# Janmajayamall/tfhe-research

Measured on AMD Instinct MI355X. Metric: programmable_bootstraps_per_sec, higher is better.
Workload: dtype f64

## Files before the change

tfhe-research_amd/csrc/pbs_wave.h:

```cpp
#pragma once
#include "wave_ntt.h"

namespace tfhe {

template <int V>
struct IntC {
  static constexpr int value = V;
};

template <int I, int END, class F>
TFHE_HD void static_for(F&& f) {
  if constexpr (I < END) {
    f(IntC<I>{});
    static_for<I + 1, END>(f);
  }
}

template <class F, int LOGN, int K>
constexpr int key_layout_e() {
  return (F::kLogShrink == 1 && LOGN == 9 && K == 1) ? 8 : 0;
}

struct PbsParams {
  u32 n;
  u32 k;
  u32 log_n;
  u32 tv_shift;
  u32 log_base;
  u32 levels;
  u32 ignored_bits;
  u32 first_shift;
  u32 acc_glwe = 0;
  u32 acc_offset = 0;
};

struct KsParams {
  u32 log_base;
  u32 levels;
  u32 ignored_bits;
  u32 first_shift;
};

TFHE_HD u32 round_value(u32 v, u32 ignored_bits) {
  if (ignored_bits == 0) return v;
  return ((v >> ignored_bits) + ((v >> (ignored_bits - 1)) & 1u)) << ignored_bits;
}

struct RoundConsts {
  u32 half, keep;
};
TFHE_HD RoundConsts round_consts(u32 ignored_bits) {
  return ignored_bits == 0 ? RoundConsts{0u, ~0u} : RoundConsts{1u << (ignored_bits - 1), ~((1u << ignored_bits) - 1u)};
}
TFHE_HD u32 round_value_fast(u32 v, RoundConsts rc) { return (v + rc.half) & rc.keep; }

TFHE_HD u32 decompose_limb(u32 v, u32 shift, u32 log_base, u32& carry) {
  const u32 res = ((v >> shift) & ((1u << log_base) - 1u)) + carry;
  const u32 carry_mask = res & (1u << (log_base - 1));
  carry = carry_mask >> (log_base - 1);
  return res - (carry_mask << 1);
}

template <bool SMALL_BASE>
TFHE_HD u32 decompose_limb_fast(u32& v, u32 shift, u32 log_base, u32 carry_width) {
  const u32 half = 1u << (log_base - 1);
#if defined(__HIP_DEVICE_COMPILE__)
  const u32 res = __builtin_amdgcn_ubfe(v, shift, log_base) + __builtin_amdgcn_ubfe(v, log_base - 1, carry_width);
  const u32 hb = res & half;
  u32 digit;
  if (SMALL_BASE) {
    asm("v_mad_i32_i24 %0, %1, -2, %2" : "=v"(digit) : "v"(hb), "v"(res));
  } else {
    digit = res - (hb << 1);
  }
  asm("v_bfi_b32 %0, %1, %2, %3" : "=v"(v) : "s"(half), "v"(res), "v"(v));
  return digit;
#else
  const u32 cin = carry_width ? ((v >> (log_base - 1)) & 1u) : 0u;
  const u32 res = ((v >> shift) & ((1u << log_base) - 1u)) + cin;
  const u32 hb = res & half;
  v = hb | (v & ~half);
  return res - (hb << 1);
#endif
}

TFHE_HD u32 switch_modulus_2n(u32 v, u32 log_n) {
  const u32 sh = 32u - (log_n + 1u);
  return ((v >> sh) + ((v >> (sh - 1u)) & 1u)) & ((2u << log_n) - 1u);
}

template <int LOGN>
TFHE_HD u32 monomial_coeff(const u32* poly, int j, u32 m) {
  constexpr int N = 1 << LOGN;
  const int deg = (int)(m & (N - 1));
  const u32 flip = (m >> LOGN) & 1u;
  const u32 v = poly[(j - deg) & (N - 1)];
  const u32 negate = flip ^ (u32)(j < deg);
  return negate ? (0u - v) : v;
}

template <class F, int LOGN, int K, int G, int KEYS, int NS, class Ctx, class Src, class Out, class EndKey>
TFHE_HD void external_product_team_multi(const Ctx& c, const PbsParams& P, const typename F::elem* ggsw,
                                         size_t ggsw_words, Src src, Out out, EndKey end_of_key) {
  typedef typename F::elem elem;
  static_assert(KEYS == 1 || NS == 1, "several keys or several samples, not both");
  constexpr int LT = LOGN - F::kLogShrink;
  constexpr int E = NttShape<LT, G>::kE;
  constexpr int EC = NttShape<LOGN, G>::kE;
  constexpr int CO = F::kCoeffs;
  static_assert(EC == E * CO, "coefficients per lane");
  constexpr int T = NttShape<LOGN, G>::kThreads;
  constexpr int N = 1 << LT;
  constexpr int PARTS = F::kParts;
  const int lane = c.tid();
  const int me = c.group();
  constexpr bool SPLIT = F::template split_accum<E>() && KEYS == 1 && NS == 1;
  constexpr int ACCS = KEYS * PARTS;

  elem accum[NS][ACCS][E];
  elem accum_lo[SPLIT ? ACCS : 1][SPLIT ? E : 1];
#pragma unroll
  for (int s = 0; s < NS; ++s)
#pragma unroll
    for (int q = 0; q < ACCS; ++q)
#pragma unroll
      for (int r = 0; r < E; ++r) {
        accum[s][q][r] = SPLIT ? F::accum_init() : F::zero();
        if (SPLIT) accum_lo[SPLIT ? q : 0][SPLIT ? r : 0] = F::zero();
      }

  TopConsts<F, LT, G, true> ftop;
  ftop.issue(c.twiddles_uniform());
  u32 v[NS][EC];
  const RoundConsts rc = round_consts(P.ignored_bits);
#pragma unroll
  for (int s = 0; s < NS; ++s)
#pragma unroll
    for (int r = 0; r < EC; ++r) v[s][r] = round_value_fast(src(s, r * T + lane), rc);
  ftop.ready();

  constexpr int kChunkRegisters = 8;
  constexpr int TILES = (K + 1) * ACCS;
  constexpr int CH_MAX = kChunkRegisters * 8 / (int)sizeof(elem) / (NS > 1 ? 2 : 1);
  constexpr int CH = E < CH_MAX ? E : CH_MAX;
  constexpr int CHUNKS = TILES * (E / CH);
  auto tile_ptr = [&](u32 level, int sp, int a) -> const elem* {
    const int m = a / PARTS, q = a % PARTS;
    if (TFHE_PROBE_HOT_KEY) return ggsw;
    return ggsw + (size_t)m * ggsw_words + (((size_t)(sp * P.levels + level) * (K + 1) + me) * PARTS + q) * N;
  };
  const bool two = NS == 1 && c.exchange_buffers() == 2;
  elem kbuf[2][CH];
  constexpr bool OWN = F::kLogShrink == 1 && NS == 1 && G == 1 && !SPLIT;
  constexpr bool OWN_REGS = OWN;
  constexpr bool LATE = OWN;
  auto source_of = [&](int sp) -> int {
    if (!OWN) return sp;
    const int at = me + sp;
    return at > K ? at - (K + 1) : at;
  };
  auto load_chunk = [&](u32 level, auto ci_c, int buf) {
    constexpr int ci = decltype(ci_c)::value;
    constexpr int PIECES = E / CH;
    constexpr int q = ci % ACCS, r0 = ((ci / ACCS) % PIECES) * CH, src_poly = ci / (ACCS * PIECES);
    const elem* tile = tile_ptr(level, source_of(src_poly), q);
#pragma unroll
    for (int r = 0; r < CH; ++r)
      kbuf[buf][r] = tile[TFHE_PROBE_HOT_KEY ? (lane & 63) + r : spectrum_slot<LT, G, (int)sizeof(elem), key_layout_e<F, LOGN, K>()>(lane, r0 + r)];
  };
  auto buffers_of_level = [&](u32 t, Ctx (&cl)[NS]) {
#pragma unroll
    for (int s = 0; s < NS; ++s) cl[s] = c.with_exchange_buffer(NS > 1 ? s : (two ? (int)(t & 1u) : 0));
  };
#pragma unroll 1
  for (u32 t = 0; t < P.levels; ++t) {
    const u32 level = P.levels - 1 - t;
    const u32 shift = P.first_shift + P.log_base * t;
    Ctx cl[NS];
    buffers_of_level(t, cl);
    static_for<0, 1>([&](auto pre_c) { load_chunk(level, pre_c, decltype(pre_c)::value); });
    c.compiler_fence();
    constexpr int FS = 1;
    const u32 carry_width = (t == 0) ? 0u : 1u;
    elem own[OWN_REGS ? NS : 1][OWN_REGS ? E : 1];
#pragma unroll
    for (int s0 = 0; s0 < NS; s0 += FS) {
      elem work[FS][E];
      if (F::kMaxLogBase <= 23 || P.log_base <= 23) {
#pragma unroll
        for (int s = 0; s < FS; ++s)
#pragma unroll
          for (int r = 0; r < E; ++r) {
            u32 dg[CO];
#pragma unroll
            for (int q = 0; q < CO; ++q) dg[q] = decompose_limb_fast<true>(v[s0 + s][r + q * E], shift, P.log_base, carry_width);
            work[s][r] = F::from_digits(dg);
          }
      } else {
#pragma unroll
        for (int s = 0; s < FS; ++s)
#pragma unroll
          for (int r = 0; r < E; ++r) {
            u32 dg[CO];
#pragma unroll
            for (int q = 0; q < CO; ++q) dg[q] = decompose_limb_fast<false>(v[s0 + s][r + q * E], shift, P.log_base, carry_width);
            work[s][r] = F::from_digits(dg);
          }
      }
      Ctx cf[FS];
#pragma unroll
      for (int s = 0; s < FS; ++s) cf[s] = cl[s0 + s];
      if constexpr (LATE) {
        ntt_forward_multi<F, LT, G, true, true>(cf, work, ftop, [&]() { if (t > 0 && !two && s0 == 0) c.team_sync(); });
      } else {
        ntt_forward_multi<F, LT, G, true, true>(cf, work, ftop);
      }
#pragma unroll
      for (int s = 0; s < FS; ++s) {
        if (F::kReduceSpectrum) {
#pragma unroll
          for (int r = 0; r < E; ++r) work[s][r] = F::reduce(work[s][r]);
        }
        elem* mine = cf[s].scratch();
#pragma unroll
        for (int r = 0; r < E; ++r) mine[exchange_slot<LT, G>(lane, r)] = work[s][r];
        if constexpr (OWN_REGS) {
#pragma unroll
          for (int r = 0; r < E; ++r) own[s0 + s][r] = work[s][r];
        }
      }
    }
    if constexpr (!OWN) c.team_sync();
    elem d[NS][CH];
    constexpr bool MAC_LOW = mac_lowers_priority<elem, E>() && KEYS == 1;
    if constexpr (MAC_LOW) wave_priority<0>();
    static_for<0, CHUNKS>([&](auto ci_c) {
      constexpr int ci = decltype(ci_c)::value;
      constexpr int PIECES = E / CH;
      constexpr int q = ci % ACCS, r0 = ((ci / ACCS) % PIECES) * CH, sp = ci / (ACCS * PIECES);
      constexpr int cur = ci % 2;
      if constexpr (OWN && ci == ACCS * PIECES) c.team_sync();
      if constexpr (ci + 1 < CHUNKS) load_chunk(level, IntC<ci + 1>{}, (ci + 1) % 2);
      if constexpr (OWN_REGS && sp == 0) {
        if constexpr (q == 0) {
#pragma unroll
          for (int s = 0; s < NS; ++s)
#pragma unroll
            for (int r = 0; r < CH; ++r) d[s][r] = own[s][r0 + r];
        }
      } else if constexpr (q == 0 && !(TFHE_PROBE_NO_EXCHANGE_READS)) {
#pragma unroll
        for (int s = 0; s < NS; ++s) {
          const elem* spec = cl[s].scratch_of(source_of(sp));
#pragma unroll
          for (int r = 0; r < CH; ++r) d[s][r] = spec[exchange_slot<LT, G>(lane, r0 + r)];
        }
      } else if constexpr (q == 0 && ci == 0) {
#pragma unroll
        for (int s = 0; s < NS; ++s)
#pragma unroll
          for (int r = 0; r < CH; ++r) d[s][r] = kbuf[0][r];
      }
      c.compiler_fence();
#pragma unroll
      for (int s = 0; s < NS; ++s)
#pragma unroll
        for (int r = 0; r < CH; ++r) {
          if (SPLIT)
            F::mac(d[s][r], kbuf[cur][r], accum[s][q][r0 + r], accum_lo[SPLIT ? q : 0][SPLIT ? r0 + r : 0]);
          else
            accum[s][q][r0 + r] = F::mul_add(d[s][r], kbuf[cur][r], accum[s][q][r0 + r]);
        }
    });
    if constexpr (MAC_LOW) wave_priority<2>();
    if (!two && !LATE) c.team_sync();
  }

  Ctx ci[NS];
  buffers_of_level(P.levels, ci);
  TopConsts<F, LT, G, false> itop;
  itop.issue(c.twiddles_uniform());
  constexpr bool PAIR = NS == 1 && PARTS == 2 && G == 1 && !SPLIT && NttShape<LT, G>::kPasses == 3 && F::kLogShrink == 1 && E == 8;
  static_for<0, KEYS>([&](auto key_c) {
    constexpr int m = decltype(key_c)::value;
    if constexpr (PAIR) {
#pragma unroll
      for (int r = 0; r < E; ++r) {
        accum[0][m * PARTS][r] = F::before_inverse(accum[0][m * PARTS][r]);
        accum[0][m * PARTS + 1][r] = F::before_inverse(accum[0][m * PARTS + 1][r]);
      }
      if constexpr (m == 0) itop.ready();
      if constexpr (LATE && m == 0)
        ntt_inverse_pair<F, LT, G>(ci[0], accum[0][m * PARTS], accum[0][m * PARTS + 1], itop, [&]() { if (!two) c.team_sync(); });
      else
        ntt_inverse_pair<F, LT, G>(ci[0], accum[0][m * PARTS], accum[0][m * PARTS + 1], itop);
    }
    static_for<0, PAIR ? 0 : PARTS>([&](auto part_c) {
      constexpr int q = m * PARTS + decltype(part_c)::value;
      elem x[NS][E];
#pragma unroll
      for (int s = 0; s < NS; ++s)
#pragma unroll
        for (int r = 0; r < E; ++r)
          x[s][r] = SPLIT ? F::mac_finish(accum[s][q][r], accum_lo[SPLIT ? q : 0][SPLIT ? r : 0])
                          : F::before_inverse(accum[s][q][r]);
      if constexpr (LATE) {
        if constexpr (q == 0) {
          itop.ready();
          ntt_inverse_multi<F, LT, G>(ci, x, itop, [&]() { if (!two) c.team_sync(); });
        } else {
          ntt_inverse_multi<F, LT, G>(ci, x, itop);
        }
      } else {
        if constexpr (q == 0) itop.ready();
        ntt_inverse_multi<F, LT, G>(ci, x, itop);
      }
#pragma unroll
      for (int s = 0; s < NS; ++s)
#pragma unroll
        for (int r = 0; r < E; ++r) accum[s][q][r] = x[s][r];
    });
#pragma unroll
    for (int s = 0; s < NS; ++s)
#pragma unroll
      for (int r = 0; r < E; ++r) {
        elem parts[PARTS];
#pragma unroll
        for (int q = 0; q < PARTS; ++q) parts[q] = accum[s][m * PARTS + q][r];
        u32 vals[CO];
        F::finish(parts, vals);
#pragma unroll
        for (int q = 0; q < CO; ++q) out(m, s, (r + q * E) * T + lane, vals[q]);
      }
    end_of_key(m);
  });
  if (two) c.team_sync();
}

template <class F, int LOGN, int K, int G, int KEYS, class Ctx, class Src, class Out, class EndKey>
TFHE_HD void external_product_team_keys(const Ctx& c, const PbsParams& P, const typename F::elem* ggsw,
                                        size_t ggsw_words, Src src, Out out, EndKey end_of_key) {
  external_product_team_multi<F, LOGN, K, G, KEYS, 1>(
      c, P, ggsw, ggsw_words, [&](int, int j) -> u32 { return src(j); },
      [&](int m, int, int j, u32 value) { out(m, j, value); }, end_of_key);
}

template <class F, int LOGN, int K, int G, class Ctx, class Src, class Out>
TFHE_HD void external_product_team(const Ctx& c, const PbsParams& P, const typename F::elem* ggsw,
                                   Src src, Out out) {
  external_product_team_keys<F, LOGN, K, G, 1>(
      c, P, ggsw, 0, src, [&](int, int j, u32 value) { out(j, value); }, [](int) {});
}

template <class F, int LOGN, int K, int G, class Ctx>
TFHE_HD void pack_lwe_team(const Ctx& c, const PbsParams& P, const u32* masks_t, u32 d, const u32* body,
                           const typename F::elem* key , u32 slice_begin, u32 slice_end) {
  constexpr int E = NttShape<LOGN, G>::kE;
  constexpr int T = NttShape<LOGN, G>::kThreads;
  constexpr int N = 1 << LOGN;
  const int lane = c.tid();
  const int me = c.group();
  u32* acc = c.acc();
#pragma unroll
  for (int r = 0; r < E; ++r) acc[r * T + lane] = (me == K && body != nullptr) ? body[r * T + lane] : 0u;
  const size_t slice_words = (size_t)(K + 1) * P.levels * (K + 1) * F::kParts * (N >> F::kLogShrink);
#pragma unroll 1
  for (u32 s = slice_begin; s < slice_end; ++s) {
    const u32 i = c.uniform(s * (u32)(K + 1) + (u32)me);
    const bool live = i < d;
    const u32* column = masks_t + (size_t)(live ? i : 0u) * N;
    auto src = [&](int j) -> u32 { return live ? column[j] : 0u; };
    auto out = [&](int j, u32 value) { c.lds_add(acc + j, 0u - value); };
    external_product_team<F, LOGN, K, G>(c, P, key + (size_t)s * slice_words, src, out);
    if (G > 1 && c.exchange_buffers() != 2) c.poly_sync();
  }
}

struct RotateInit {
  int deg;
  u32 flip;
};
template <int LOGN>
TFHE_HD RotateInit rotate_init(const PbsParams& P, u32 body) {
  constexpr u32 N = 1u << LOGN;
  const u32 b_tilde = switch_modulus_2n(body, LOGN);
  const u32 m = (2u * N - b_tilde + 2u * N - P.acc_offset) & (2u * N - 1u);
  return RotateInit{(int)(m & (N - 1)), (m >> LOGN) & 1u};
}
template <int LOGN>
TFHE_HD u32 rotate_init_word(const RotateInit& ri, const u32* poly, int j, u32 shift) {
  constexpr int N = 1 << LOGN;
  const u32 t = poly[(j - ri.deg) & (N - 1)] << shift;
  return (ri.flip ^ (u32)(j < ri.deg)) ? (0u - t) : t;
}
template <int LOGN, int K, int COUNT, class Index>
TFHE_HD void rotate_init_fill(const PbsParams& P, const RotateInit& ri, const u32* tv, int me, u32* acc, Index index) {
  constexpr int N = 1 << LOGN;
  if (P.acc_glwe) {
    const u32* mine = tv + (size_t)me * N;
#pragma unroll
    for (int r = 0; r < COUNT; ++r) acc[index(r)] = rotate_init_word<LOGN>(ri, mine, index(r), 0u);
  } else {
#pragma unroll
    for (int r = 0; r < COUNT; ++r) acc[index(r)] = me == K ? rotate_init_word<LOGN>(ri, tv, index(r), P.tv_shift) : 0u;
  }
}

template <class F, int LOGN, int K, int G, int NS, class Ctx>
TFHE_HD void blind_rotate_team_multi(const Ctx& c, const PbsParams& P, const u32* const* lwe ,
                                     const u32* const* tv ,
                                     const typename F::elem* bsk , u32 i_begin, u32 i_end,
                                     const u32* const* resume ) {
  constexpr int E = NttShape<LOGN, G>::kE;
  constexpr int T = NttShape<LOGN, G>::kThreads;
  constexpr int N = 1 << LOGN;
  const int lane = c.tid();
  const int me = c.group();

  if (i_begin > 0) {
#pragma unroll
    for (int s = 0; s < NS; ++s) {
      u32* acc = c.acc(s);
      const u32* from = resume[s] + (size_t)me * N;
#pragma unroll
      for (int r = 0; r < E; ++r) acc[r * T + lane] = from[r * T + lane];
    }
  } else {
#pragma unroll
  for (int s = 0; s < NS; ++s) {
    u32* acc = c.acc(s);
    const RotateInit ri = rotate_init<LOGN>(P, lwe[s][P.n]);
    rotate_init_fill<LOGN, K, E>(P, ri, tv[s], me, acc, [&](int r) { return r * T + lane; });
  }
  }
  c.poly_sync();

  const size_t ggsw_words = (size_t)(K + 1) * P.levels * (K + 1) * F::kParts * (N >> F::kLogShrink);
#pragma unroll 1
  for (u32 i = i_begin; i < i_end; ++i) {
    u32 a_tilde[NS];
#pragma unroll
    for (int s = 0; s < NS; ++s) a_tilde[s] = c.uniform(switch_modulus_2n(lwe[s][i], LOGN));
    auto src = [&](int s, int j) -> u32 {
      const u32* acc = c.acc(s);
      return monomial_coeff<LOGN>(acc, j, a_tilde[s]) - acc[j];
    };
    auto out = [&](int, int s, int j, u32 value) { c.lds_add(c.acc(s) + j, value); };
    external_product_team_multi<F, LOGN, K, G, 1, NS>(c, P, bsk + (size_t)i * ggsw_words, 0, src, out, [](int) {});
    if (NS > 1 || c.exchange_buffers() != 2) c.poly_sync();
  }
}

template <class F, int LOGN, int K, int G, int NS, class Ctx>
TFHE_HD void blind_rotate_team_multi(const Ctx& c, const PbsParams& P, const u32* const* lwe, const u32* const* tv,
                                     const typename F::elem* bsk) {
  blind_rotate_team_multi<F, LOGN, K, G, NS>(c, P, lwe, tv, bsk, 0u, P.n, nullptr);
}

template <class F, int LOGN, int K, int G, class Ctx>
TFHE_HD void blind_rotate_team(const Ctx& c, const PbsParams& P, const u32* lwe ,
                               const u32* tv ,
                               const typename F::elem* bsk ) {
  const u32* const lwes[1] = {lwe};
  const u32* const tvs[1] = {tv};
  blind_rotate_team_multi<F, LOGN, K, G, 1>(c, P, lwes, tvs, bsk);
}

template <class F, int LOGN, int K, int LEVELS, int RING>
struct WideKeyRing {
  static constexpr int E = NttShape<LOGN - 1, 1>::kE;
  static constexpr int R = (K + 1) * LEVELS;
  static constexpr int kRing = RING;
  static_assert(LEVELS > 0 && RING > 0 && R % RING == 0, "the ring holds a divisor of the product's rows");
  typename F::elem slot[RING][E];
  template <int M>
  TFHE_HD void load(const typename F::elem* ggsw, int me, int q, int lane) {
    constexpr int level = M / (K + 1), sp = M % (K + 1);
    const typename F::elem* tile = ggsw + ((((size_t)sp * LEVELS + level) * (K + 1) + me) * 2 + q) * ((size_t)1 << (LOGN - 1));
#pragma unroll
    for (int r = 0; r < E; ++r)
      slot[M % RING][r] = tile[spectrum_slot<LOGN - 1, 1, (int)sizeof(typename F::elem), key_layout_e<F, LOGN, K>()>(lane, r)];
  }
  TFHE_HD void prime(const typename F::elem* ggsw, int me, int q, int lane) {
    static_for<0, RING>([&](auto m_c) { load<decltype(m_c)::value>(ggsw, me, q, lane); });
  }
};
struct NoKeyRing {
  static constexpr int kRing = 1;
};
constexpr int largest_divisor_upto(int n, int cap) {
  int best = 1;
  for (int d = 1; d <= n && d <= cap; ++d)
    if (n % d == 0) best = d;
  return best;
}
template <int LOGN, int K, int LEVELS>
constexpr int wide_ring_rows() {
  constexpr int E = NttShape<LOGN - 1, 1>::kE;
  return LEVELS == 0 ? 0 : largest_divisor_upto((K + 1) * LEVELS, (K == 1 ? 224 : 112) / (4 * E));
}


template <class F, int LOGN, int K, int LEVELS = 0, class Ring = NoKeyRing, class Ctx, class Src, class Out>
TFHE_HD void external_product_team_wide(const Ctx& c, const PbsParams& P, const typename F::elem* ggsw,
                                        const typename F::elem* ggsw_next, Ring& ring, Src src, Out out) {
  typedef typename F::elem elem;
  static_assert(F::kParts == 2 && F::kLogShrink == 1 && F::kCoeffs == 2, "the complex transform: two key parts, two coefficients per element");
  constexpr int LT = LOGN - 1;
  constexpr int E = NttShape<LT, 1>::kE;
  constexpr int EC = 2 * E;
  constexpr int T = 64;
  constexpr int N = 1 << LT;
  constexpr bool RINGED = LEVELS > 0;
  const int lane = c.tid();
  const int me = c.group();
  const int q = c.half();
  const u32 levels = RINGED ? (u32)LEVELS : P.levels;
  const u32 split = (levels + 1u) / 2u;
  const u32 t_begin = q == 0 ? 0u : split, t_end = q == 0 ? split : levels;

  TopConsts<F, LT, 1, true> ftop;
  ftop.issue(c.twiddles_uniform());
  u32 v[EC];
  const RoundConsts rc = round_consts(P.ignored_bits);
#pragma unroll
  for (int r = 0; r < EC; ++r) v[r] = round_value_fast(src(r * T + lane), rc);
  ftop.ready();

  constexpr int CH0 = E < 4 ? E : 4;
  constexpr int CH = (((K + 1) * (E / CH0)) % 2 == 0) ? CH0 : CH0 / 2;
  constexpr int PIECES = E / CH;
  constexpr int CHK = (K + 1) * PIECES;
  elem kbuf[RINGED ? 1 : 2][RINGED ? 1 : CH];
  auto load_chunk = [&](u32 level, auto ci_c, int buf) {
    constexpr int ci = decltype(ci_c)::value;
    constexpr int sp = ci / PIECES, r0 = (ci % PIECES) * CH;
    const elem* tile = ggsw + ((((size_t)sp * levels + level) * (K + 1) + me) * 2 + q) * N;
#pragma unroll
    for (int r = 0; r < CH; ++r)
      kbuf[RINGED ? 0 : buf][RINGED ? 0 : r] = tile[spectrum_slot<LT, 1, (int)sizeof(elem), key_layout_e<F, LOGN, K>()>(lane, r0 + r)];
  };
  if constexpr (!RINGED) {
    load_chunk(0u, IntC<0>{}, 0);
    c.compiler_fence();
  }

#pragma unroll 1
  for (u32 t = 0; t < t_end; ++t) {
    const u32 shift = P.first_shift + P.log_base * t;
    const u32 carry_width = (t == 0) ? 0u : 1u;
    elem work[E];
#pragma unroll
    for (int r = 0; r < E; ++r) {
      u32 dg[2];
      dg[0] = decompose_limb_fast<true>(v[r], shift, P.log_base, carry_width);
      dg[1] = decompose_limb_fast<true>(v[r + E], shift, P.log_base, carry_width);
      work[r] = F::from_digits(dg);
    }
    if (t < t_begin) continue;
    const u32 row = (u32)me * levels + (levels - 1u - t);
    ntt_forward<F, LT, 1, true, true>(c, work, ftop);
    elem* published = c.row_buffer((int)row);
#pragma unroll
    for (int r = 0; r < E; ++r) published[exchange_slot<LT, 1>(lane, r)] = work[r];
  }
  TopConsts<F, LT, 1, false> itop;
  itop.issue(c.twiddles_uniform());
  c.team_sync();

  elem accum[E];
#pragma unroll
  for (int r = 0; r < E; ++r) accum[r] = F::zero();
  if constexpr (RINGED) {
    constexpr int R = (K + 1) * LEVELS;
    constexpr int RING_ROWS = Ring::kRing;
    static_for<0, R>([&](auto m_c) {
      constexpr int m = decltype(m_c)::value;
      constexpr int level = m / (K + 1), sp = m % (K + 1);
      const elem* spec = c.row_buffer(sp * LEVELS + level);
      elem d[E];
#pragma unroll
      for (int r = 0; r < E; ++r) d[r] = spec[exchange_slot<LT, 1>(lane, r)];
#pragma unroll
      for (int r = 0; r < E; ++r) accum[r] = F::mul_add(d[r], ring.slot[m % RING_ROWS][r], accum[r]);
      c.compiler_fence();
      if constexpr (m + RING_ROWS < R) ring.template load<m + RING_ROWS>(ggsw, me, q, lane);
      else ring.template load<m + RING_ROWS - R>(ggsw_next, me, q, lane);
    });
  } else {
#pragma unroll 1
    for (u32 level = 0; level < levels; ++level) {
      static_for<0, CHK>([&](auto ci_c) {
        constexpr int ci = decltype(ci_c)::value;
        constexpr int sp = ci / PIECES, r0 = (ci % PIECES) * CH;
        constexpr int cur = ci % 2;
        static_assert(CHK % 2 == 0, "an even number of chunks per level keeps the buffer parity static");
        if constexpr (ci + 1 < CHK) {
          load_chunk(level, IntC<ci + 1>{}, (ci + 1) % 2);
        } else {
          if (level + 1u < levels) load_chunk(level + 1u, IntC<0>{}, 0);
        }
        const elem* spec = c.row_buffer((int)((u32)sp * levels + level));
        elem d[CH];
#pragma unroll
        for (int r = 0; r < CH; ++r) d[r] = spec[exchange_slot<LT, 1>(lane, r0 + r)];
        c.compiler_fence();
#pragma unroll
        for (int r = 0; r < CH; ++r) accum[r0 + r] = F::mul_add(d[r], kbuf[RINGED ? 0 : cur][RINGED ? 0 : r], accum[r0 + r]);
      });
    }
  }

#pragma unroll
  for (int r = 0; r < E; ++r) accum[r] = F::before_inverse(accum[r]);
  itop.ready();
  ntt_inverse<F, LT, 1>(c, accum, itop);
#pragma unroll
  for (int r = 0; r < E; ++r) {
    out(q, r * T + lane, F::to_u32(accum[r].re));
    out(q, (r + E) * T + lane, F::to_u32(accum[r].im));
  }
}

template <class F, int LOGN, int K, int LEVELS = 0, int RING = 0, class Ctx>
TFHE_HD void blind_rotate_team_wide(const Ctx& c, const PbsParams& P, const u32* lwe , const u32* tv ,
                                    const typename F::elem* bsk , u32 i_begin, u32 i_end,
                                    const u32* resume ) {
  constexpr int N = 1 << LOGN;
  constexpr int EC = N / 64;
  const int lane = c.tid();
  const int me = c.group();
  const int q = c.half();
  u32* acc = c.acc();
  const u32 levels = LEVELS > 0 ? (u32)LEVELS : P.levels;
  const size_t ggsw_words = (size_t)(K + 1) * levels * (K + 1) * 2 * (N >> 1);
  typename std::conditional<(LEVELS > 0), WideKeyRing<F, LOGN, K, (LEVELS > 0 ? LEVELS : 1), (RING > 0 ? RING : 1)>, NoKeyRing>::type ring;
  if constexpr (LEVELS > 0) {
    if (i_begin < i_end) ring.prime(bsk + (size_t)i_begin * ggsw_words, me, q, lane);
  }
  if (i_begin > 0) {
    const u32* from = resume + (size_t)me * N;
#pragma unroll
    for (int r = 0; r < EC / 2; ++r) acc[(r + q * (EC / 2)) * 64 + lane] = from[(r + q * (EC / 2)) * 64 + lane];
  } else {
    const RotateInit ri = rotate_init<LOGN>(P, lwe[P.n]);
    rotate_init_fill<LOGN, K, EC / 2>(P, ri, tv, me, acc, [&](int r) { return (r + q * (EC / 2)) * 64 + lane; });
  }
  c.team_sync();
#pragma unroll 1
  for (u32 i = i_begin; i < i_end; ++i) {
    const u32 a_tilde = c.uniform(switch_modulus_2n(lwe[i], LOGN));
    auto src = [&](int j) -> u32 { return monomial_coeff<LOGN>(acc, j, a_tilde) - acc[j]; };
    auto out = [&](int half, int j, u32 value) { c.lds_add(acc + j, value << (16 * half)); };
    const typename F::elem* ggsw = bsk + (size_t)i * ggsw_words;
    const typename F::elem* ggsw_next = i + 1 < i_end ? ggsw + ggsw_words : ggsw;
    external_product_team_wide<F, LOGN, K, LEVELS>(c, P, ggsw, ggsw_next, ring, src, out);
    c.team_sync();
  }
}

template <class F, int LOGN, class Ctx, class Src, class Out>
TFHE_HD void external_product_pair(const Ctx& c, const PbsParams& P, const typename F::elem* ggsw, Src src, Out out) {
  typedef typename F::elem elem;
  static_assert(F::kParts == 2 && F::kLogShrink == 1 && F::kCoeffs == 2, "the complex transform: two key parts, two coefficients per element");
  constexpr int K = 1;
  constexpr int LT = LOGN - 1;
  constexpr int G = 0;
  constexpr int E = NttShape<LT, G>::kE;
  constexpr int EC = 2 * E;
  constexpr int T = NttShape<LT, G>::kThreads;
  constexpr int N = 1 << LT;
  const int tid = c.tid();
  const int me = c.group();

  elem accum[2][E];
#pragma unroll
  for (int q = 0; q < 2; ++q)
#pragma unroll
    for (int r = 0; r < E; ++r) accum[q][r] = F::zero();

  TopConsts<F, LT, G, true> ftop;
  ftop.issue(c.twiddles_uniform());
  u32 v[EC];
  const RoundConsts rc = round_consts(P.ignored_bits);
#pragma unroll
  for (int r = 0; r < EC; ++r) v[r] = round_value_fast(src(r * T + tid), rc);
  ftop.ready();

  constexpr int CH = 4;
  constexpr int PIECES = E / CH;
  constexpr int CHUNKS = 2 * PIECES * 2;
  elem kbuf[2][CH];
  constexpr int KEY_E = key_layout_e<F, LOGN, 1>();
  static_assert(KEY_E == E, "the prepared key of the pair shape has the pair kernel's layout");
  auto load_chunk = [&](u32 level, auto ci_c, int buf) {
    constexpr int ci = decltype(ci_c)::value;
    constexpr int q = ci % 2, r0 = ((ci / 2) % PIECES) * CH, other = ci / (2 * PIECES);
    const int sp = other ? 1 - me : me;
    const elem* tile = ggsw + ((((size_t)sp * P.levels + level) * (K + 1) + me) * 2 + q) * N;
#pragma unroll
    for (int r = 0; r < CH; ++r) kbuf[buf][r] = tile[spectrum_slot<LT, G, (int)sizeof(elem), KEY_E>(tid, r0 + r)];
  };
#pragma unroll 1
  for (u32 t = 0; t < P.levels; ++t) {
    const u32 level = P.levels - 1 - t;
    const u32 shift = P.first_shift + P.log_base * t;
    const u32 carry_width = (t == 0) ? 0u : 1u;
    load_chunk(level, IntC<0>{}, 0);
    c.compiler_fence();
    elem work[E];
#pragma unroll
    for (int r = 0; r < E; ++r) {
      u32 dg[2];
      dg[0] = decompose_limb_fast<true>(v[r], shift, P.log_base, carry_width);
      dg[1] = decompose_limb_fast<true>(v[r + E], shift, P.log_base, carry_width);
      work[r] = F::from_digits(dg);
    }
    ntt_forward<F, LT, G, true, true>(c, work, ftop);
    elem* mine = c.scratch();
#pragma unroll
    for (int r = 0; r < E; ++r) mine[exchange_slot<LT, G>(tid, r)] = work[r];
    c.wave_sync();
    elem d[CH];
    static_for<0, CHUNKS>([&](auto ci_c) {
      constexpr int ci = decltype(ci_c)::value;
      constexpr int q = ci % 2, r0 = ((ci / 2) % PIECES) * CH, other = ci / (2 * PIECES);
      if constexpr (ci + 1 < CHUNKS) load_chunk(level, IntC<ci + 1>{}, (ci + 1) % 2);
      if constexpr (q == 0) {
        if constexpr (other == 0) {
#pragma unroll
          for (int r = 0; r < CH; ++r) d[r] = work[r0 + r];
        } else {
          const elem* spec = c.scratch_of(1 - me);
#pragma unroll
          for (int r = 0; r < CH; ++r) d[r] = spec[exchange_slot<LT, G>(tid, r0 + r)];
        }
      }
      c.compiler_fence();
#pragma unroll
      for (int r = 0; r < CH; ++r) accum[q][r0 + r] = F::mul_add(d[r], kbuf[ci % 2][r], accum[q][r0 + r]);
    });
    c.wave_sync();
  }

  TopConsts<F, LT, G, false> itop;
  itop.issue(c.twiddles_uniform());
#pragma unroll
  for (int r = 0; r < E; ++r) {
    accum[0][r] = F::before_inverse(accum[0][r]);
    accum[1][r] = F::before_inverse(accum[1][r]);
  }
  itop.ready();
  ntt_inverse_pair<F, LT, G>(c, accum[0], accum[1], itop);
#pragma unroll
  for (int r = 0; r < E; ++r) {
    elem parts[2] = {accum[0][r], accum[1][r]};
    u32 vals[2];
    F::finish(parts, vals);
    out(r * T + tid, vals[0]);
    out((r + E) * T + tid, vals[1]);
  }
}

template <class F, int LOGN, class Ctx>
TFHE_HD void blind_rotate_pair(const Ctx& c, const PbsParams& P, const u32* lwe , const u32* tv ,
                               const typename F::elem* bsk , u32 i_begin, u32 i_end,
                               const u32* resume ) {
  constexpr int N = 1 << LOGN;
  constexpr int T = 32;
  constexpr int EC = N / T;
  constexpr int K = 1;
  const int tid = c.tid();
  const int me = c.group();
  u32* acc = c.acc();
  if (i_begin > 0) {
    const u32* from = resume + (size_t)me * N;
#pragma unroll
    for (int r = 0; r < EC; ++r) acc[r * T + tid] = from[r * T + tid];
  } else {
    const RotateInit ri = rotate_init<LOGN>(P, lwe[P.n]);
    rotate_init_fill<LOGN, K, EC>(P, ri, tv, me, acc, [&](int r) { return r * T + tid; });
  }
  c.wave_sync();
  const size_t ggsw_words = (size_t)(K + 1) * P.levels * (K + 1) * 2 * (N >> 1);
#pragma unroll 1
  for (u32 i = i_begin; i < i_end; ++i) {
    const u32 a_tilde = c.uniform(switch_modulus_2n(lwe[i], LOGN));
    auto src = [&](int j) -> u32 { return monomial_coeff<LOGN>(acc, j, a_tilde) - acc[j]; };
    auto out = [&](int j, u32 value) { c.lds_add(acc + j, value); };
    external_product_pair<F, LOGN>(c, P, bsk + (size_t)i * ggsw_words, src, out);
    c.wave_sync();
  }
}

template <class F, int LOGN, int K, int G, class Ctx>
TFHE_HD void blind_rotate_bmmp_team(const Ctx& c, const PbsParams& P, const u32* lwe ,
                                    const u32* tv ,
                                    const typename F::elem* bsk ) {
  constexpr int E = NttShape<LOGN, G>::kE;
  constexpr int T = NttShape<LOGN, G>::kThreads;
  constexpr int N = 1 << LOGN;
  const int lane = c.tid();
  const int me = c.group();
  u32* acc = c.acc(0);
  {
    const u32 b_tilde = switch_modulus_2n(lwe[P.n], LOGN);
    const u32 m = (2u * N - b_tilde) & (2u * N - 1u);
    const int deg = (int)(m & (N - 1));
    const u32 flip = (m >> LOGN) & 1u;
#pragma unroll
    for (int r = 0; r < E; ++r) {
      const int j = r * T + lane;
      u32 val = 0;
      if (me == K) {
        const u32 t = tv[(j - deg) & (N - 1)] << P.tv_shift;
        val = (flip ^ (u32)(j < deg)) ? (0u - t) : t;
      }
      acc[j] = val;
    }
    c.poly_sync();
  }
  const size_t ggsw_words = (size_t)(K + 1) * P.levels * (K + 1) * F::kParts * (N >> F::kLogShrink);
  u32* stage = reinterpret_cast<u32*>(c.scratch());
#pragma unroll 1
  for (u32 pair = 0; pair < P.n / 2; ++pair) {
    const u32 a0 = c.uniform(switch_modulus_2n(lwe[2 * pair], LOGN));
    const u32 a1 = c.uniform(switch_modulus_2n(lwe[2 * pair + 1], LOGN));
    const u32 e[3] = {(a0 + a1) & (2u * N - 1u), a0, a1};
    auto src = [&](int j) -> u32 { return acc[j]; };
    auto out = [&](int, int j, u32 value) { stage[j] = value; };
    auto end_of_key = [&](int m) {
      c.poly_sync();
#pragma unroll
      for (int r = 0; r < E; ++r) {
        const int j = r * T + lane;
        acc[j] += monomial_coeff<LOGN>(stage, j, e[m]) - stage[j];
      }
      c.poly_sync();
    };
    external_product_team_keys<F, LOGN, K, G, 3>(c, P, bsk + (size_t)pair * 3 * ggsw_words, ggsw_words, src, out,
                                                 end_of_key);
    if (c.exchange_buffers() != 2) c.poly_sync();
  }
}

template <int LOGN, int K, int G, class Ctx>
TFHE_HD void sample_extract_team(const Ctx& c, u32* out , int s = 0) {
  constexpr int E = NttShape<LOGN, G>::kE;
  constexpr int T = NttShape<LOGN, G>::kThreads;
  constexpr int N = 1 << LOGN;
  const int lane = c.tid();
  const int me = c.group();
  const u32* acc = c.acc(s);
  if (me < K) {
#pragma unroll
    for (int r = 0; r < E; ++r) {
      const int x = r * T + lane;
      out[me * N + x] = (x == 0) ? acc[0] : (0u - acc[N - x]);
    }
  } else if (lane == 0) {
    out[K * N] = acc[0];
  }
}

struct CmuxTreePass {
  const void* selectors;
  const void* rot_selectors;
  size_t query_stride;
  u32 tables;
  u32 height;
  u32 log_subtrees;
  u32 shared_sets;
  const u32* even;
  const u32* odd;
  size_t pair_stride, set_stride;
  const u32* table;
  size_t table_stride;
  u32 log_entries;
  u32 rot_steps;
  u32* pending;
  u32* glwe_out;
  u32* lwe_out;
};

template <class F, int LOGN, int K, int G, class Ctx>
TFHE_HD void cmux_tree_team(const Ctx& c, const PbsParams& P, const CmuxTreePass& A, size_t tree, u32 subtree) {
  typedef typename F::elem elem;
  constexpr int E = NttShape<LOGN, G>::kE;
  constexpr int T = NttShape<LOGN, G>::kThreads;
  constexpr int N = 1 << LOGN;
  constexpr size_t GLWE = (size_t)(K + 1) * N;
  const int lane = c.tid();
  const int me = c.group();
  u32* acc = c.acc();
  const size_t ggsw_words = (size_t)(K + 1) * P.levels * (K + 1) * F::kParts * (N >> F::kLogShrink);
  const size_t query = tree / A.tables;
  const size_t set = A.shared_sets ? tree % A.tables : tree;
  const elem* sel = static_cast<const elem*>(A.selectors) + query * A.query_stride;
  const elem* rot = static_cast<const elem*>(A.rot_selectors) + query * A.query_stride;
  const size_t team = (tree << A.log_subtrees) + subtree;
  u32* pending = A.height > 1 ? A.pending + team * (A.height - 1) * GLWE + (size_t)me * N : nullptr;
  const bool from_table = A.even == nullptr;
  const u32* tab = from_table ? A.table + set * A.table_stride : nullptr;
  const u32 entries = 1u << A.log_entries;
  const size_t leaf0 = (size_t)subtree << A.height;
  auto table_word = [&](size_t leaf, int j) -> u32 {
    return (me == K && (u32)j < entries) ? tab[(leaf << A.log_entries) + (u32)j] << P.tv_shift : 0u;
  };

  if (A.height == 0) {
    const u32* only = from_table ? nullptr : A.even + set * A.set_stride + (size_t)me * N;
#pragma unroll
    for (int r = 0; r < E; ++r) acc[r * T + lane] = from_table ? table_word(leaf0, r * T + lane) : only[r * T + lane];
  }
  const u32 tree_products = A.height ? (1u << A.height) - 1u : 0u;
  const u32 products = tree_products + A.rot_steps;
  if (products > tree_products && tree_products == 0) c.poly_sync();
  u32 p = 0, t = 0;
#pragma unroll 1
  for (u32 step = 0; step < products; ++step) {
    const bool rotating = step >= tree_products;
    const bool at_leaves = !rotating && t == 0;
    const size_t pair = (leaf0 >> 1) + p;
    const size_t leaf_at = set * A.set_stride + pair * A.pair_stride + (size_t)me * N;
    const u32* a = rotating ? nullptr : !at_leaves ? pending + (size_t)(t - 1) * GLWE : from_table ? nullptr : A.even + leaf_at;
    const u32* b = (at_leaves && !from_table) ? A.odd + leaf_at : nullptr;
    const u32 m = c.uniform(2u * N - (1u << (rotating ? step - tree_products : 0u)));
    auto src = [&](int j) -> u32 {
      if (rotating) return monomial_coeff<LOGN>(acc, j, m) - acc[j];
      if (!at_leaves) return acc[j] - a[j];
      if (from_table) return table_word(2 * pair + 1, j) - table_word(2 * pair, j);
      return b[j] - a[j];
    };
    auto out = [&](int j, u32 value) {
      if (rotating) c.lds_add(acc + j, value);
      else if (at_leaves && from_table) acc[j] = table_word(2 * pair, j) + value;
      else acc[j] = a[j] + value;
    };
    external_product_team<F, LOGN, K, G>(c, P, (rotating ? rot + (size_t)(step - tree_products) * ggsw_words : sel + (size_t)t * ggsw_words), src, out);
    if (c.exchange_buffers() != 2) c.poly_sync();
    if (!rotating) {
      ++t;
      if (!((p >> (t - 1)) & 1u)) {
        if (t < A.height) {
          u32* slot = pending + (size_t)(t - 1) * GLWE;
#pragma unroll
          for (int r = 0; r < E; ++r) slot[r * T + lane] = acc[r * T + lane];
        }
        ++p;
        t = 0;
      }
    }
  }
  if (A.glwe_out) {
    u32* dst = A.glwe_out + team * GLWE + (size_t)me * N;
#pragma unroll
    for (int r = 0; r < E; ++r) dst[r * T + lane] = acc[r * T + lane];
  }
  if (A.lwe_out) {
    c.poly_sync();
    sample_extract_team<LOGN, K, G>(c, A.lwe_out + team * ((size_t)K * N + 1));
  }
}

TFHE_HD void global_add(u32* p, u32 v) {
#if defined(__HIP_DEVICE_COMPILE__)
  atomicAdd(p, v);
#else
  __atomic_fetch_add(p, v, __ATOMIC_RELAXED);
#endif
}

struct DemuxTreePass {
  const void* selectors;
  const void* rot_selectors;
  size_t query_stride;
  u32 values;
  u32 height;
  u32 log_subtrees;
  u32 shared_sets;
  u32 rot_steps;
  u32 accumulate;
  const u32* roots;
  u32* pending;
  u32* leaves;
  size_t set_stride;
};

template <class F, int LOGN, int K, int G, class Ctx>
TFHE_HD void demux_tree_team(const Ctx& c, const PbsParams& P, const DemuxTreePass& A, size_t tree, u32 subtree) {
  typedef typename F::elem elem;
  constexpr int E = NttShape<LOGN, G>::kE;
  constexpr int T = NttShape<LOGN, G>::kThreads;
  constexpr int N = 1 << LOGN;
  constexpr size_t GLWE = (size_t)(K + 1) * N;
  const int lane = c.tid();
  const int me = c.group();
  u32* acc = c.acc();
  const size_t ggsw_words = (size_t)(K + 1) * P.levels * (K + 1) * F::kParts * (N >> F::kLogShrink);
  const size_t query = tree / A.values;
  const size_t set = A.shared_sets ? tree % A.values : tree;
  const elem* sel = static_cast<const elem*>(A.selectors) + query * A.query_stride;
  const elem* rot = static_cast<const elem*>(A.rot_selectors) + query * A.query_stride;
  const size_t team = (tree << A.log_subtrees) + subtree;
  u32* pending = A.height > 1 ? A.pending + team * (A.height - 1) * GLWE + (size_t)me * N : nullptr;
  u32* leaves = A.leaves + set * A.set_stride + ((size_t)subtree << A.height) * GLWE + (size_t)me * N;
  const bool adding = A.accumulate != 0;
  auto emit = [&](u32* dst, u32 value) {
    if (adding) global_add(dst, value);
    else *dst = value;
  };

  const u32* root = A.roots + team * GLWE + (size_t)me * N;
#pragma unroll
  for (int r = 0; r < E; ++r) acc[r * T + lane] = root[r * T + lane];
  const u32 tree_products = A.height ? (1u << A.height) - 1u : 0u;
  const u32 products = A.rot_steps + tree_products;
  if (A.rot_steps) c.poly_sync();
  u32 t = A.height, node = 0;
#pragma unroll 1
  for (u32 step = 0; step < products; ++step) {
    const bool rotating = step < A.rot_steps;
    const bool last_level = !rotating && t == 1;
    const u32 m = c.uniform(1u << (rotating ? step : 0u));
    u32* slot = (rotating || last_level) ? nullptr : pending + (size_t)(t - 2) * GLWE;
    u32* left = last_level ? leaves + (size_t)(2 * node) * GLWE : nullptr;
    auto src = [&](int j) -> u32 {
      if (rotating) return monomial_coeff<LOGN>(acc, j, m) - acc[j];
      return acc[j];
    };
    auto out = [&](int j, u32 value) {
      if (rotating) {
        c.lds_add(acc + j, value);
      } else if (last_level) {
        emit(left + GLWE + j, value);
        emit(left + j, acc[j] - value);
      } else {
        slot[j] = acc[j] - value;
        acc[j] = value;
      }
    };
    external_product_team<F, LOGN, K, G>(c, P, (rotating ? rot + (size_t)step * ggsw_words : sel + (size_t)(t - 1) * ggsw_words), src, out);
    if (c.exchange_buffers() != 2) c.poly_sync();
    if (rotating) continue;
    if (!last_level) {
      node = 2 * node + 1;
      --t;
    } else if (node != 0) {
      const u32 up = (u32)__builtin_ctz(node);
      node = (node >> up) - 1u;
      t = up + 1u;
      const u32* parked = pending + (size_t)(t - 1) * GLWE;
#pragma unroll
      for (int r = 0; r < E; ++r) acc[r * T + lane] = parked[r * T + lane];
    }
  }
  if (A.height == 0) {
#pragma unroll
    for (int r = 0; r < E; ++r) emit(leaves + r * T + lane, acc[r * T + lane]);
  }
}

struct ProgramOp {
  u32 sel, lo, hi, rot;
  u32 dst;
};

struct CmuxProgramPass {
  const void* selectors;
  size_t query_stride;
  const ProgramOp* ops;
  const u32* outputs;
  const u32* terminals;
  u32 n_terminals;
  u32 n_nodes;
  u32 n_outputs;
  u32 parts;
  u32 op_begin, op_end;
  u32 out_begin, out_end;
  u32* values;
  u32* glwe_out;
  u32* lwe_out;
};

template <class F, int LOGN, int K, int G, class Ctx>
TFHE_HD void cmux_program_team(const Ctx& c, const PbsParams& P, const CmuxProgramPass& A, size_t query, u32 part) {
  typedef typename F::elem elem;
  constexpr int E = NttShape<LOGN, G>::kE;
  constexpr int T = NttShape<LOGN, G>::kThreads;
  constexpr int N = 1 << LOGN;
  constexpr size_t GLWE = (size_t)(K + 1) * N;
  const int lane = c.tid();
  const int me = c.group();
  u32* acc = c.acc();
  const size_t ggsw_words = (size_t)(K + 1) * P.levels * (K + 1) * F::kParts * (N >> F::kLogShrink);
  const elem* sel = static_cast<const elem*>(A.selectors) + query * A.query_stride;
  u32* values = A.values + query * A.n_nodes * GLWE + (size_t)me * N;
  const u32 nt = A.n_terminals;
  const bool body = me == K;
  auto word = [&](u32 ref, int j) -> u32 {
    if (ref < nt) return body ? A.terminals[(size_t)ref * N + j] << P.tv_shift : 0u;
    return values[(size_t)(ref - nt) * GLWE + j];
  };

  const u32 op_share = (A.op_end - A.op_begin + A.parts - 1) / A.parts;
  const u32 op_first = A.op_begin + part * op_share;
  const u32 op_last = op_first + op_share < A.op_end ? op_first + op_share : A.op_end;
#pragma unroll 1
  for (u32 i = op_first; i < op_last; ++i) {
    const u32 lo = c.uniform(A.ops[i].lo), hi = c.uniform(A.ops[i].hi), rot = c.uniform(A.ops[i].rot);
    u32* dst = values + (size_t)c.uniform(A.ops[i].dst) * GLWE;
    if (rot) {
#pragma unroll
      for (int r = 0; r < E; ++r) acc[r * T + lane] = word(hi, r * T + lane);
      c.poly_sync();
    }
    auto src = [&](int j) -> u32 { return (rot ? monomial_coeff<LOGN>(acc, j, rot) : word(hi, j)) - word(lo, j); };
    auto out = [&](int j, u32 value) { dst[j] = word(lo, j) + value; };
    external_product_team<F, LOGN, K, G>(c, P, sel + (size_t)c.uniform(A.ops[i].sel) * ggsw_words, src, out);
    if (c.exchange_buffers() != 2) c.poly_sync();
  }

  const u32 out_share = (A.out_end - A.out_begin + A.parts - 1) / A.parts;
  const u32 out_first = A.out_begin + part * out_share;
  const u32 out_last = out_first + out_share < A.out_end ? out_first + out_share : A.out_end;
#pragma unroll 1
  for (u32 o = out_first; o < out_last; ++o) {
    const u32 ref = c.uniform(A.outputs[o]);
    const size_t at = query * A.n_outputs + o;
    if (A.glwe_out) {
      u32* dst = A.glwe_out + at * GLWE + (size_t)me * N;
#pragma unroll
      for (int r = 0; r < E; ++r) dst[r * T + lane] = word(ref, r * T + lane);
    }
    if (A.lwe_out) {
#pragma unroll
      for (int r = 0; r < E; ++r) acc[r * T + lane] = word(ref, r * T + lane);
      c.poly_sync();
      sample_extract_team<LOGN, K, G>(c, A.lwe_out + at * ((size_t)K * N + 1));
      c.poly_sync();
    }
  }
}

template <class F, int LOGN, int G, int LAYOUT_E = 0, class Ctx>
TFHE_HD void bsk_prepare_wave(const Ctx& c, const u32* poly, typename F::elem* spec ,
                              typename F::elem n_inv) {
  typedef typename F::elem elem;
  constexpr int LT = LOGN - F::kLogShrink;
  constexpr int E = NttShape<LT, G>::kE;
  constexpr int CO = F::kCoeffs;
  constexpr int T = NttShape<LOGN, G>::kThreads;
  constexpr int NS = 1 << LT;
  const int lane = c.tid();
#pragma unroll 1
  for (int part = 0; part < F::kParts; ++part) {
    elem x[E];
#pragma unroll
    for (int r = 0; r < E; ++r) {
      u32 w[CO];
#pragma unroll
      for (int q = 0; q < CO; ++q) w[q] = poly[(r + q * E) * T + lane];
      x[r] = F::from_key_words(w, part);
    }
    ntt_forward<F, LT, G>(c, x);
#pragma unroll
    for (int r = 0; r < E; ++r) spec[(size_t)part * NS + spectrum_slot<LT, G, (int)sizeof(elem), LAYOUT_E>(lane, r)] = F::scale_key(x[r], n_inv);
  }
}

template <class F, int LOGN, int G, class Ctx, class Out>
TFHE_HD void glwe_mask_dot_key(const Ctx& c, u32 k, const u32* masks ,
                               const u32* sk , typename F::elem n_inv, Out out) {
  typedef typename F::elem elem;
  constexpr int LT = LOGN - F::kLogShrink;
  constexpr int E = NttShape<LT, G>::kE;
  constexpr int CO = F::kCoeffs;
  constexpr int T = NttShape<LOGN, G>::kThreads;
  constexpr int N = 1 << LOGN;
  constexpr int PARTS = F::kParts;
  const int lane = c.tid();

  elem accum[PARTS][E];
#pragma unroll
  for (int q = 0; q < PARTS; ++q)
#pragma unroll
    for (int r = 0; r < E; ++r) accum[q][r] = F::zero();

#pragma unroll 1
  for (u32 i = 0; i < k; ++i) {
    elem s[E];
#pragma unroll
    for (int r = 0; r < E; ++r) {
      u32 w[CO];
#pragma unroll
      for (int q = 0; q < CO; ++q) w[q] = sk[(size_t)i * N + (r + q * E) * T + lane];
      s[r] = F::from_digits(w);
    }
    ntt_forward<F, LT, G, true>(c, s);
#pragma unroll
    for (int r = 0; r < E; ++r) s[r] = F::scale_key(s[r], n_inv);
    static_for<0, PARTS>([&](auto part_c) {
      constexpr int q = decltype(part_c)::value;
      elem x[E];
#pragma unroll
      for (int r = 0; r < E; ++r) {
        u32 w[CO];
#pragma unroll
        for (int qq = 0; qq < CO; ++qq) w[qq] = masks[(size_t)i * N + (r + qq * E) * T + lane];
        x[r] = F::from_key_words(w, q);
      }
      ntt_forward<F, LT, G>(c, x);
#pragma unroll
      for (int r = 0; r < E; ++r)
        accum[q][r] = F::mul_add(F::kReduceSpectrum ? F::reduce(x[r]) : x[r], s[r], accum[q][r]);
    });
  }

  static_for<0, PARTS>([&](auto part_c) {
    constexpr int q = decltype(part_c)::value;
#pragma unroll
    for (int r = 0; r < E; ++r) accum[q][r] = F::before_inverse(accum[q][r]);
    ntt_inverse<F, LT, G>(c, accum[q]);
  });
#pragma unroll
  for (int r = 0; r < E; ++r) {
    elem parts[PARTS];
#pragma unroll
    for (int q = 0; q < PARTS; ++q) parts[q] = accum[q][r];
    u32 vals[CO];
    F::finish(parts, vals);
#pragma unroll
    for (int q = 0; q < CO; ++q) out((r + q * E) * T + lane, vals[q]);
  }
}

}
```

Before: 143,100.

## Precompute rotation sign mask and keep decomposition carries in registers

Replaces the per-coefficient monomial rotation lambda with a RotatingOperand that precomputes, per lane, a bitmask of which coefficients get negated and two LDS base pointers. This removes index masking, comparison and negation branches from the rounding load. It also carries the signed-digit decomposition carry in a register between levels and uses bitfield-extract and xad instructions instead of recomputing the carry from shifted bits. The cost is one extra register per coefficient, inline asm that relies on LDS address-space casts, and a more complex selection of code paths through SFINAE.

```diff
diff --git a/tfhe-research_amd/csrc/pbs_wave.h b/tfhe-research_amd/csrc/pbs_wave.h
--- a/tfhe-research_amd/csrc/pbs_wave.h
+++ b/tfhe-research_amd/csrc/pbs_wave.h
@@ -1,4 +1,6 @@
 #pragma once
+#include <utility>
+
 #include "wave_ntt.h"
 
 namespace tfhe {
@@ -84,6 +86,32 @@
 #endif
 }
 
+TFHE_HD u32 bit_field(u32 v, u32 shift, u32 width) {
+#if defined(__HIP_DEVICE_COMPILE__)
+  return __builtin_amdgcn_ubfe(v, shift, width);
+#else
+  return (v >> shift) & ((1u << width) - 1u);
+#endif
+}
+template <bool CARRY_IN>
+TFHE_HD u32 decompose_limb_reg(u32 v, u32 shift, u32 log_base, u32 half, u32& carry) {
+  u32 res = bit_field(v, shift, log_base);
+  if (CARRY_IN) res += carry;
+  carry = bit_field(res, log_base - 1, 1);
+#if defined(__HIP_DEVICE_COMPILE__)
+  u32 digit;
+  asm("v_xad_u32 %0, %1, %2, %3" : "=v"(digit) : "v"(res), "s"(half), "v"(0u - half));
+  return digit;
+#else
+  return (res ^ half) - half;
+#endif
+}
+
+template <class F, int LOGN, int K, int G, int NS>
+constexpr bool short_hot_loop() {
+  return F::kLogShrink == 1 && G == 1 && ((K == 1 && NS == 1) || (LOGN == 9 && K == 2));
+}
+
 TFHE_HD u32 switch_modulus_2n(u32 v, u32 log_n) {
   const u32 sh = 32u - (log_n + 1u);
   return ((v >> sh) + ((v >> (sh - 1u)) & 1u)) & ((2u << log_n) - 1u);
@@ -97,6 +125,78 @@
   const u32 v = poly[(j - deg) & (N - 1)];
   const u32 negate = flip ^ (u32)(j < deg);
   return negate ? (0u - v) : v;
+}
+
+template <int LOGN, int T>
+struct RotatingOperand {
+  static constexpr int N = 1 << LOGN;
+  static constexpr int kCount = N / T;
+  static_assert(kCount <= 32 && (T & (T - 1)) == 0, "one bit per coefficient; T a power of two");
+#if defined(__HIP_DEVICE_COMPILE__)
+  typedef const __attribute__((address_space(3))) u32* LdsWords;
+  typedef u32 Words;
+  TFHE_HD static Words words_at(const u32* p) { return (u32)(size_t)(LdsWords)p; }
+  TFHE_HD static u32 read(Words negated, Words kept, u32 s, int index) {
+    return ((LdsWords)(size_t)((negated & s) | (kept & ~s)))[index];
+  }
+#else
+  typedef const u32* Words;
+  TFHE_HD static Words words_at(const u32* p) { return p; }
+  TFHE_HD static u32 read(Words negated, Words kept, u32 s, int index) { return (s ? negated : kept)[index]; }
+#endif
+  const u32* own;
+  Words negated, kept;
+  u32 signs;
+  TFHE_HD RotatingOperand() {}
+  TFHE_HD RotatingOperand(const u32* acc, int lane, u32 m) {
+    const int deg = (int)(m & (u32)(N - 1));
+    const bool flip = ((m >> LOGN) & 1u) != 0;
+    int log_t = 0;
+    while ((1 << log_t) < T) ++log_t;
+    const int k = (deg - lane + (T - 1)) >> log_t;
+    own = acc + lane;
+    const u32* base = own - deg;
+    negated = words_at(base + (flip ? 0 : N));
+    kept = words_at(base + (flip ? N : 0));
+    signs = (u32)(~0ull << k) ^ (flip ? 0u : ~0u);
+  }
+  TFHE_HD u32 rounded(int r, RoundConsts rc) const {
+    u32 s = (u32)((int)(signs << (31 - r)) >> 31);
+#if defined(__HIP_DEVICE_COMPILE__)
+    asm("" : "+v"(s));
+#endif
+    const u32 c = (rc.half - own[r * T]) - s;
+    return ((read(negated, kept, s, r * T) ^ s) + c) & rc.keep;
+  }
+};
+template <int LOGN, int T, int NS>
+struct RotatingOperands {
+  const RotatingOperand<LOGN, T>* of;
+  TFHE_HD u32 rounded(int s, int r, RoundConsts rc) const { return of[s].rounded(r, rc); }
+};
+template <class Src, class = u32>
+struct reads_rounded : std::false_type {};
+template <class Src>
+struct reads_rounded<Src, decltype(std::declval<const Src&>().rounded(0, 0, RoundConsts{}))> : std::true_type {};
+template <class Src, class = u32>
+struct reads_rounded1 : std::false_type {};
+template <class Src>
+struct reads_rounded1<Src, decltype(std::declval<const Src&>().rounded(0, RoundConsts{}))> : std::true_type {};
+template <int T, class Src>
+TFHE_HD auto rounded_coeff(const Src& src, int s, int r, int, RoundConsts rc, int) -> decltype(src.rounded(s, r, rc)) {
+  return src.rounded(s, r, rc);
+}
+template <int T, class Src>
+TFHE_HD u32 rounded_coeff(const Src& src, int s, int r, int lane, RoundConsts rc, long) {
+  return round_value_fast(src(s, r * T + lane), rc);
+}
+template <int T, class Src>
+TFHE_HD auto rounded_coeff(const Src& src, int r, int, RoundConsts rc, int) -> decltype(src.rounded(r, rc)) {
+  return src.rounded(r, rc);
+}
+template <int T, class Src>
+TFHE_HD u32 rounded_coeff(const Src& src, int r, int lane, RoundConsts rc, long) {
+  return round_value_fast(src(r * T + lane), rc);
 }
 
 template <class F, int LOGN, int K, int G, int KEYS, int NS, class Ctx, class Src, class Out, class EndKey>
@@ -129,14 +229,16 @@
         if (SPLIT) accum_lo[SPLIT ? q : 0][SPLIT ? r : 0] = F::zero();
       }
 
+  constexpr bool CARRY_REG = reads_rounded<Src>::value;
   TopConsts<F, LT, G, true> ftop;
   ftop.issue(c.twiddles_uniform());
-  u32 v[NS][EC];
+  u32 v[NS][EC], carry[NS][CARRY_REG ? EC : 1];
   const RoundConsts rc = round_consts(P.ignored_bits);
+  const u32 half_base = 1u << (P.log_base - 1);
 #pragma unroll
   for (int s = 0; s < NS; ++s)
 #pragma unroll
-    for (int r = 0; r < EC; ++r) v[s][r] = round_value_fast(src(s, r * T + lane), rc);
+    for (int r = 0; r < EC; ++r) v[s][r] = rounded_coeff<T>(src, s, r, lane, rc, 0);
   ftop.ready();
 
   constexpr int kChunkRegisters = 8;
@@ -186,6 +288,29 @@
 #pragma unroll
     for (int s0 = 0; s0 < NS; s0 += FS) {
       elem work[FS][E];
+      if constexpr (CARRY_REG) {
+        if (t == 0) {
+#pragma unroll
+          for (int s = 0; s < FS; ++s)
+#pragma unroll
+            for (int r = 0; r < E; ++r) {
+              u32 dg[CO];
+#pragma unroll
+              for (int q = 0; q < CO; ++q) dg[q] = decompose_limb_reg<false>(v[s0 + s][r + q * E], shift, P.log_base, half_base, carry[s0 + s][CARRY_REG ? r + q * E : 0]);
+              work[s][r] = F::from_digits(dg);
+            }
+        } else {
+#pragma unroll
+          for (int s = 0; s < FS; ++s)
+#pragma unroll
+            for (int r = 0; r < E; ++r) {
+              u32 dg[CO];
+#pragma unroll
+              for (int q = 0; q < CO; ++q) dg[q] = decompose_limb_reg<true>(v[s0 + s][r + q * E], shift, P.log_base, half_base, carry[s0 + s][CARRY_REG ? r + q * E : 0]);
+              work[s][r] = F::from_digits(dg);
+            }
+        }
+      } else {
       if (F::kMaxLogBase <= 23 || P.log_base <= 23) {
 #pragma unroll
         for (int s = 0; s < FS; ++s)
@@ -206,6 +331,7 @@
             for (int q = 0; q < CO; ++q) dg[q] = decompose_limb_fast<false>(v[s0 + s][r + q * E], shift, P.log_base, carry_width);
             work[s][r] = F::from_digits(dg);
           }
+      }
       }
       Ctx cf[FS];
 #pragma unroll
@@ -446,7 +572,14 @@
       return monomial_coeff<LOGN>(acc, j, a_tilde[s]) - acc[j];
     };
     auto out = [&](int, int s, int j, u32 value) { c.lds_add(c.acc(s) + j, value); };
-    external_product_team_multi<F, LOGN, K, G, 1, NS>(c, P, bsk + (size_t)i * ggsw_words, 0, src, out, [](int) {});
+    if constexpr (short_hot_loop<F, LOGN, K, G, NS>()) {
+      RotatingOperand<LOGN, T> rotated[NS];
+#pragma unroll
+      for (int s = 0; s < NS; ++s) rotated[s] = RotatingOperand<LOGN, T>(c.acc(s), lane, a_tilde[s]);
+      external_product_team_multi<F, LOGN, K, G, 1, NS>(c, P, bsk + (size_t)i * ggsw_words, 0, RotatingOperands<LOGN, T, NS>{rotated}, out, [](int) {});
+    } else {
+      external_product_team_multi<F, LOGN, K, G, 1, NS>(c, P, bsk + (size_t)i * ggsw_words, 0, src, out, [](int) {});
+    }
     if (NS > 1 || c.exchange_buffers() != 2) c.poly_sync();
   }
 }
@@ -521,10 +654,12 @@
 
   TopConsts<F, LT, 1, true> ftop;
   ftop.issue(c.twiddles_uniform());
-  u32 v[EC];
+  constexpr bool CARRY_REG = reads_rounded1<Src>::value;
+  u32 v[EC], carry[CARRY_REG ? EC : 1];
   const RoundConsts rc = round_consts(P.ignored_bits);
-#pragma unroll
-  for (int r = 0; r < EC; ++r) v[r] = round_value_fast(src(r * T + lane), rc);
+  const u32 half_base = 1u << (P.log_base - 1);
+#pragma unroll
+  for (int r = 0; r < EC; ++r) v[r] = rounded_coeff<T>(src, r, lane, rc, 0);
   ftop.ready();
 
   constexpr int CH0 = E < 4 ? E : 4;
@@ -548,14 +683,34 @@
 #pragma unroll 1
   for (u32 t = 0; t < t_end; ++t) {
     const u32 shift = P.first_shift + P.log_base * t;
-    const u32 carry_width = (t == 0) ? 0u : 1u;
     elem work[E];
-#pragma unroll
-    for (int r = 0; r < E; ++r) {
-      u32 dg[2];
-      dg[0] = decompose_limb_fast<true>(v[r], shift, P.log_base, carry_width);
-      dg[1] = decompose_limb_fast<true>(v[r + E], shift, P.log_base, carry_width);
-      work[r] = F::from_digits(dg);
+    if constexpr (CARRY_REG) {
+      if (t == 0) {
+#pragma unroll
+        for (int r = 0; r < E; ++r) {
+          u32 dg[2];
+          dg[0] = decompose_limb_reg<false>(v[r], shift, P.log_base, half_base, carry[CARRY_REG ? r : 0]);
+          dg[1] = decompose_limb_reg<false>(v[r + E], shift, P.log_base, half_base, carry[CARRY_REG ? r + E : 0]);
+          work[r] = F::from_digits(dg);
+        }
+      } else {
+#pragma unroll
+        for (int r = 0; r < E; ++r) {
+          u32 dg[2];
+          dg[0] = decompose_limb_reg<true>(v[r], shift, P.log_base, half_base, carry[CARRY_REG ? r : 0]);
+          dg[1] = decompose_limb_reg<true>(v[r + E], shift, P.log_base, half_base, carry[CARRY_REG ? r + E : 0]);
+          work[r] = F::from_digits(dg);
+        }
+      }
+    } else {
+      const u32 carry_width = (t == 0) ? 0u : 1u;
+#pragma unroll
+      for (int r = 0; r < E; ++r) {
+        u32 dg[2];
+        dg[0] = decompose_limb_fast<true>(v[r], shift, P.log_base, carry_width);
+        dg[1] = decompose_limb_fast<true>(v[r + E], shift, P.log_base, carry_width);
+        work[r] = F::from_digits(dg);
+      }
     }
     if (t < t_begin) continue;
     const u32 row = (u32)me * levels + (levels - 1u - t);
@@ -654,7 +809,11 @@
     auto out = [&](int half, int j, u32 value) { c.lds_add(acc + j, value << (16 * half)); };
     const typename F::elem* ggsw = bsk + (size_t)i * ggsw_words;
     const typename F::elem* ggsw_next = i + 1 < i_end ? ggsw + ggsw_words : ggsw;
-    external_product_team_wide<F, LOGN, K, LEVELS>(c, P, ggsw, ggsw_next, ring, src, out);
+    if constexpr (short_hot_loop<F, LOGN, K, 1, 1>()) {
+      external_product_team_wide<F, LOGN, K, LEVELS>(c, P, ggsw, ggsw_next, ring, RotatingOperand<LOGN, 64>(acc, lane, a_tilde), out);
+    } else {
+      external_product_team_wide<F, LOGN, K, LEVELS>(c, P, ggsw, ggsw_next, ring, src, out);
+    }
     c.team_sync();
   }
 }
@@ -681,10 +840,11 @@
 
   TopConsts<F, LT, G, true> ftop;
   ftop.issue(c.twiddles_uniform());
-  u32 v[EC];
+  u32 v[EC], carry[EC];
   const RoundConsts rc = round_consts(P.ignored_bits);
-#pragma unroll
-  for (int r = 0; r < EC; ++r) v[r] = round_value_fast(src(r * T + tid), rc);
+  const u32 half_base = 1u << (P.log_base - 1);
+#pragma unroll
+  for (int r = 0; r < EC; ++r) v[r] = rounded_coeff<T>(src, r, tid, rc, 0);
   ftop.ready();
 
   constexpr int CH = 4;
@@ -705,16 +865,25 @@
   for (u32 t = 0; t < P.levels; ++t) {
     const u32 level = P.levels - 1 - t;
     const u32 shift = P.first_shift + P.log_base * t;
-    const u32 carry_width = (t == 0) ? 0u : 1u;
     load_chunk(level, IntC<0>{}, 0);
     c.compiler_fence();
     elem work[E];
-#pragma unroll
-    for (int r = 0; r < E; ++r) {
-      u32 dg[2];
-      dg[0] = decompose_limb_fast<true>(v[r], shift, P.log_base, carry_width);
-      dg[1] = decompose_limb_fast<true>(v[r + E], shift, P.log_base, carry_width);
-      work[r] = F::from_digits(dg);
+    if (t == 0) {
+#pragma unroll
+      for (int r = 0; r < E; ++r) {
+        u32 dg[2];
+        dg[0] = decompose_limb_reg<false>(v[r], shift, P.log_base, half_base, carry[r]);
+        dg[1] = decompose_limb_reg<false>(v[r + E], shift, P.log_base, half_base, carry[r + E]);
+        work[r] = F::from_digits(dg);
+      }
+    } else {
+#pragma unroll
+      for (int r = 0; r < E; ++r) {
+        u32 dg[2];
+        dg[0] = decompose_limb_reg<true>(v[r], shift, P.log_base, half_base, carry[r]);
+        dg[1] = decompose_limb_reg<true>(v[r + E], shift, P.log_base, half_base, carry[r + E]);
+        work[r] = F::from_digits(dg);
+      }
     }
     ntt_forward<F, LT, G, true, true>(c, work, ftop);
     elem* mine = c.scratch();
@@ -786,7 +955,7 @@
 #pragma unroll 1
   for (u32 i = i_begin; i < i_end; ++i) {
     const u32 a_tilde = c.uniform(switch_modulus_2n(lwe[i], LOGN));
-    auto src = [&](int j) -> u32 { return monomial_coeff<LOGN>(acc, j, a_tilde) - acc[j]; };
+    const RotatingOperand<LOGN, T> src(acc, tid, a_tilde);
     auto out = [&](int j, u32 value) { c.lds_add(acc + j, value); };
     external_product_pair<F, LOGN>(c, P, bsk + (size_t)i * ggsw_words, src, out);
     c.wave_sync();
```

Result: faster. 145,400, median of 6 (+1.6%).
